# zxhuang1698/ZeroShape

Measured on AMD Instinct MI355X. Metric: sdf_query_points_per_sec_vox128, higher is better.
Workload: dtype f16x3

## Files before the change

### zeroshape_amd/csrc/sdf_decoder_split.hip

```cpp
#include "zs_common.h"
#include <stdlib.h>
#include "sdf_layout.h"
#include "sdf_math.h"
#include "zs_split16.h"
#include "sdf_query.h"
#include "../../include/zeroshape_hip.h"

#include <math.h>
#include <stdint.h>
#include <type_traits>

namespace {

using namespace zs::lay;
using namespace zs::qry;
using zs::dm::gelu_erf;
using zs::dm::softplus100;

typedef float f32x16 __attribute__((ext_vector_type(16)));
typedef float f32x4 __attribute__((ext_vector_type(4)));
typedef float f32x2 __attribute__((ext_vector_type(2)));
typedef unsigned u32x4 __attribute__((ext_vector_type(4)));

constexpr float S_GUARD = 64.0f;
constexpr int KB_U4 = 128;
constexpr int CK = 8;
constexpr int KPW = CK / WAVES;
constexpr int CHUNK_BYTES = CK * KB_U4 * 16;
constexpr int NBUF = 2;
constexpr int KB_TOTAL = G_TOTAL / 2;
constexpr int PRM_WINDOW = 4096;
constexpr int STAGE_FLOATS = NBUF * CHUNK_BYTES / 4;
constexpr int SLAB_TILES = NT - 1;
constexpr int SLAB_U4 = SLAB_TILES * 4 * 64;
constexpr int ZTILES_F4 = NT * 4 * 64;
static_assert(ZSLAB_F4 == 3 * ZTILES_F4, "the workspace slab holds three skip layers' feat partial products");
static_assert(B0_TABLE_FLOATS == PRM_WINDOW, "block0_window_kernel / block0_stream_kernel index an image's table by PRM_WINDOW");
constexpr int LDS_FLOATS = PRM_WINDOW + STAGE_FLOATS + WAVES * SLAB_U4 * 4;
static_assert(LDS_FLOATS * 4 == 160 * 1024, "the kernel owns the whole LDS of a CU");
static_assert(KB_TOTAL % CK == 0 && CK % WAVES == 0 && KPW * 2048 <= 4096, "chunking");
static_assert((RING * GROUP_FLOATS + PARAM_FLOATS) * 4 >= NBUF * CHUNK_BYTES, "prefetch stays inside the program");

constexpr int W_PP = P_PP;
constexpr int W_BLK = P_BLK0;
constexpr int W_IA = P_LNFG;
constexpr int W_IB = P_IMPL_PAIR + P_IMPL_PAIR_STRIDE;
static_assert(P_BLK_STRIDE <= PRM_WINDOW && W_IB - W_IA <= PRM_WINDOW && P_USED - W_IB <= PRM_WINDOW,
              "params windows");

#define DEV __device__ __forceinline__

DEV void pin(u32x4 &a, u32x4 &b) { asm volatile("" : "+v"(a), "+v"(b) : : "memory"); }

using zs::s16::mfma3;
using zs::s16::split2;

struct PT {
    u32x4 v[4];
};
template <typename T>
DEV PT pack_tile(const T &x) {
    PT p;
#pragma unroll
    for (int j = 0; j < 2; j++)
#pragma unroll
        for (int i = 0; i < 4; i++) {
            unsigned h, l;
            split2(x[8 * j + 2 * i], x[8 * j + 2 * i + 1], h, l);
            p.v[2 * j][i] = h;
            p.v[2 * j + 1][i] = l;
        }
    return p;
}

DEV void glds_kblocks(const char *gsrc, unsigned lds_dst) {
#ifdef ZS_EXP_NO_DMA
    if (gsrc != nullptr) return;
#endif
    asm volatile("s_mov_b32 m0, %1\n\ts_nop 0\n\tglobal_load_lds_dwordx4 %0, off"
                 "\n\tglobal_load_lds_dwordx4 %0, off offset:1024"
                 "\n\tglobal_load_lds_dwordx4 %0, off offset:2048"
                 "\n\tglobal_load_lds_dwordx4 %0, off offset:3072"
                 :
                 : "v"(gsrc), "s"(lds_dst)
                 : "memory");
}

struct AStream {
    const u32x4 *buf[NBUF];
    unsigned dst[NBUF];
    u32x4 hi, lo;
    const char *gsrc;

    DEV void init(const char *prog, u32x4 *stage, unsigned stage_addr, int wave, int lane) {
        const char *g = prog + wave * (KPW * KB_U4 * 16) + lane * 16;
        asm volatile("s_waitcnt vmcnt(0) lgkmcnt(0)\n\ts_barrier" ::: "memory");
#pragma unroll
        for (int i = 0; i < NBUF; i++) {
            buf[i] = stage + i * (CK * KB_U4) + lane;
            dst[i] = stage_addr + i * CHUNK_BYTES + wave * (KPW * KB_U4 * 16);
            glds_kblocks(g + i * CHUNK_BYTES, dst[i]);
        }
        gsrc = g + NBUF * CHUNK_BYTES;
        asm volatile("s_waitcnt vmcnt(4)\n\ts_barrier" ::: "memory");
        hi = buf[0][0];
        lo = buf[0][64];
    }
    template <int EXTRA_VM = 0>
    DEV void step(int pos, u32x4 &ahi, u32x4 &alo) {
        ahi = hi;
        alo = lo;
        if (pos == CK - 1) {
            static_assert(EXTRA_VM == 0 || EXTRA_VM == 4, "wait-count variants");
            if (EXTRA_VM == 4)
                asm volatile("s_waitcnt vmcnt(4) lgkmcnt(0)\n\ts_barrier" ::: "memory");
            else
                asm volatile("s_waitcnt vmcnt(0) lgkmcnt(0)\n\ts_barrier" ::: "memory");
            glds_kblocks(gsrc, dst[0]);
            gsrc += CHUNK_BYTES;
            const u32x4 *t = buf[0];
            const unsigned u = dst[0];
            buf[0] = buf[1];
            dst[0] = dst[1];
            buf[1] = t;
            dst[1] = u;
            hi = buf[0][0];
            lo = buf[0][64];
        } else {
#ifndef ZS_EXP_NO_AREAD
            hi = buf[0][(pos + 1) * KB_U4];
            lo = buf[0][(pos + 1) * KB_U4 + 64];
#endif
        }
    }
    DEV void seek(const char *base, int wave, int lane) { gsrc = base + wave * (KPW * KB_U4 * 16) + lane * 16; }
    DEV void drain() { asm volatile("s_waitcnt vmcnt(0) lgkmcnt(0)" ::: "memory"); }
};

struct Slab {
    u32x4 *fl;
    PT t7;
    DEV void store(int tile, const PT &p) {
        if (tile == SLAB_TILES) {
            t7 = p;
        } else {
#pragma unroll
            for (int q = 0; q < 4; q++) fl[(tile * 4 + q) * 64] = p.v[q];
        }
    }
};

DEV f32x16 zero16() {
    f32x16 v;
#pragma unroll
    for (int r = 0; r < 16; r++) v[r] = 0.f;
    return v;
}

struct NoSide {
    DEV void operator()(int, int) const {}
};
template <typename SIDE>
DEV void mfma3_gaps(f32x16 &acc, const u32x4 &ahi, const u32x4 &alo, const u32x4 &bhi, const u32x4 &blo, int kb,
                    SIDE &side) {
    using zs::s16::as_h;
    if (std::is_same<SIDE, NoSide>::value) {
        mfma3(acc, ahi, alo, bhi, blo);
        return;
    }
    acc = __builtin_amdgcn_mfma_f32_32x32x16_f16(as_h(alo), as_h(bhi), acc, 0, 0, 0);
    side(kb, 0);
    acc = __builtin_amdgcn_mfma_f32_32x32x16_f16(as_h(ahi), as_h(blo), acc, 0, 0, 0);
    side(kb, 1);
    acc = __builtin_amdgcn_mfma_f32_32x32x16_f16(as_h(ahi), as_h(bhi), acc, 0, 0, 0);
    side(kb, 2);
}

struct TilePacker {
    PT p;
    float prev;
    DEV void feed(int kb, float v) {
        if (kb & 1) {
            unsigned h, l;
            split2(prev, v, h, l);
            p.v[2 * (kb >> 3)][(kb & 7) >> 1] = h;
            p.v[2 * (kb >> 3) + 1][(kb & 7) >> 1] = l;
        }
        prev = v;
    }
};

struct GeluStager {
    float x, u, q, t, e, p;
    DEV void s0(float v) {
        x = v;
        u = fabsf(v) * 0.70710678118654752440f;
        q = (u * u) * -1.44269504088896340736f;
    }
    DEV void s1() { t = __builtin_amdgcn_rcpf(fmaf(0.3275911f, u, 1.0f)); }
    DEV void s2() {
        e = __builtin_amdgcn_exp2f(q);
        p = fmaf(0.75052702f, t, -1.02753365f);
    }
    DEV void s3() {
        p = fmaf(p, t, 1.00509130f);
        p = fmaf(p, t, -0.20116957f);
        p = fmaf(p, t, 0.18019173f);
        p = p * t;
        u = u * p;
    }
    DEV float s4() const { return fmaf(-u, e, fmaxf(x, 0.0f)); }
    DEV float all(float v) {
        s0(v); s1(); s2(); s3();
        return s4();
    }
    DEV void stage(int st, float v, int idx, TilePacker &pk) {
        if (st == 0) s0(v);
        else if (st == 1) s1();
        else if (st == 2) s2();
        else if (st == 3) s3();
        else if (st == 4) pk.feed(idx, s4());
    }
};
struct SoftplusStager {
    float x, t;
    DEV void s0(float v) {
        x = v;
        t = __builtin_amdgcn_exp2f(fabsf(v) * -144.26950408889634074f);
    }
    DEV void s1() { t = __builtin_amdgcn_logf(1.0f + t); }
    DEV float s2() const { return fmaf(t, 0.0069314718055994530942f, fmaxf(x, 0.0f)); }
};

#ifndef ZS_EXP_TWO_TERM
#define ZS_KBLOCK_MFMA_LO_HI "v_mfma_f32_32x32x16_f16 %[acc], %[alo], %[bh], %[acc]\n\t"
#else
#define ZS_KBLOCK_MFMA_LO_HI
#endif
#define ZS_KBLOCK_GELU(NAME, BREG, LEAD) \
DEV float NAME(f32x16 &acc, const u32x4 &ahi, const u32x4 &alo, const u32x4 &bhi, const u32x4 &blo, float x) {             \
    float u, q, d, t, e, m, p;                                                                                             \
    const float c0 = 0.70710678118654752440f, c1 = 0.3275911f, c2 = -1.02753365f;                                          \
    asm volatile(                                                                                                          \
                 LEAD ZS_KBLOCK_MFMA_LO_HI                                                                                 \
                 "v_mul_f32_e64 %[u], |%[x]|, %[c0]\n\t"                                                                   \
                 "v_mul_f32_e32 %[q], %[u], %[u]\n\t"                                                                      \
                 "v_mul_f32_e32 %[q], 0xbfb8aa3b, %[q]\n\t"                                                                \
                 "v_fma_f32 %[d], %[u], %[c1], 1.0\n\t"                                                                    \
                 "v_mfma_f32_32x32x16_f16 %[acc], %[ahi], %[bl], %[acc]\n\t"                                               \
                 "v_rcp_f32_e32 %[t], %[d]\n\t"                                                                            \
                 "v_exp_f32_e32 %[e], %[q]\n\t"                                                                            \
                 "v_max_f32_e32 %[m], 0, %[x]\n\t"                                                                         \
                 "v_mfma_f32_32x32x16_f16 %[acc], %[ahi], %[bh], %[acc]\n\t"                                               \
                 "v_fmamk_f32 %[p], %[t], 0x3f40228a, %[c2]\n\t"                                                           \
                 "v_fmaak_f32 %[p], %[p], %[t], 0x3f80a6d5\n\t"                                                            \
                 "v_fmaak_f32 %[p], %[p], %[t], 0xbe4dff65\n\t"                                                            \
                 "v_fmaak_f32 %[p], %[p], %[t], 0x3e38842e\n\t"                                                            \
                 "v_mul_f32_e64 %[p], %[t], -%[p]\n\t"                                                                     \
                 "v_mul_f32_e32 %[p], %[u], %[p]\n\t"                                                                      \
                 "v_fmac_f32_e32 %[m], %[p], %[e]"                                                                         \
                 : [acc] "+v"(acc), [u] "=&v"(u), [q] "=&v"(q), [d] "=&v"(d), [t] "=&v"(t), [e] "=&v"(e), [m] "=&v"(m),    \
                   [p] "=&v"(p)                                                                                            \
                 : [alo] "v"(alo), [ahi] "v"(ahi), [bh] BREG(bhi), [bl] BREG(blo), [x] "v"(x), [c0] "s"(c0), [c1] "s"(c1), \
                   [c2] "v"(c2));                                                                                          \
    return m;                                                                                                              \
}
ZS_KBLOCK_GELU(kblock_gelu, "v", "")
ZS_KBLOCK_GELU(kblock_gelu_breg, "a", "s_nop 1\n\t")
#undef ZS_KBLOCK_GELU
#undef ZS_KBLOCK_MFMA_LO_HI
DEV float kblock_softplus(f32x16 &acc, const u32x4 &ahi, const u32x4 &alo, const u32x4 &bhi, const u32x4 &blo, float x) {
    float t, m;
    const float c0 = -144.26950408889634074f;
    asm volatile(
#ifndef ZS_EXP_TWO_TERM
                 "v_mfma_f32_32x32x16_f16 %[acc], %[alo], %[bh], %[acc]\n\t"
#endif
                 "v_mul_f32_e64 %[t], |%[x]|, %[c0]\n\t"
                 "v_exp_f32_e32 %[t], %[t]\n\t"
                 "v_mfma_f32_32x32x16_f16 %[acc], %[ahi], %[bl], %[acc]\n\t"
                 "v_max_f32_e32 %[m], 0, %[x]\n\t"
                 "v_add_f32_e32 %[t], 1.0, %[t]\n\t"
                 "v_log_f32_e32 %[t], %[t]\n\t"
                 "v_mfma_f32_32x32x16_f16 %[acc], %[ahi], %[bh], %[acc]\n\t"
                 "s_nop 0\n\t"
                 "v_fmac_f32_e32 %[m], 0x3be32166, %[t]"
                 : [acc] "+v"(acc), [t] "=&v"(t), [m] "=&v"(m)
                 : [alo] "v"(alo), [ahi] "v"(ahi), [bh] "v"(bhi), [bl] "v"(blo), [x] "v"(x), [c0] "s"(c0));
    return m;
}

DEV void mfma_settle(f32x16 &acc) { asm volatile("s_nop 7\n\ts_nop 3" : "+v"(acc)); }

template <int KT, int EXTRA_VM = 0, typename SIDE = NoSide>
DEV void gemm_reg(AStream &s, const PT *X, f32x16 &acc, SIDE side = SIDE()) {
#pragma unroll
    for (int kt = 0; kt < KT; kt++)
#pragma unroll
        for (int j = 0; j < 2; j++) {
            u32x4 ahi, alo;
            s.step((kt * 2 + j) & (CK - 1), ahi, alo);
            pin(ahi, alo);
            mfma3_gaps(acc, ahi, alo, X[kt].v[2 * j], X[kt].v[2 * j + 1], kt * 2 + j, side);
        }
}
template <typename SIDE>
DEV void mfma3_breg(f32x16 &acc, const u32x4 &ahi, const u32x4 &alo, const u32x4 &bhi, const u32x4 &blo, int kb,
                    SIDE &side) {
    asm volatile("s_nop 1\n\tv_mfma_f32_32x32x16_f16 %0, %1, %2, %0" : "+v"(acc) : "v"(alo), "a"(bhi));
    side(kb, 0);
    asm volatile("s_nop 1\n\tv_mfma_f32_32x32x16_f16 %0, %1, %2, %0" : "+v"(acc) : "v"(ahi), "a"(blo));
    side(kb, 1);
    asm volatile("s_nop 1\n\tv_mfma_f32_32x32x16_f16 %0, %1, %2, %0" : "+v"(acc) : "v"(ahi), "a"(bhi));
    side(kb, 2);
}
template <int KT, typename SIDE = NoSide>
DEV void gemm_areg(AStream &s, const PT *X, f32x16 &acc, SIDE side = SIDE()) {
#pragma unroll
    for (int kt = 0; kt < KT; kt++)
#pragma unroll
        for (int j = 0; j < 2; j++) {
            u32x4 ahi, alo;
            s.step((kt * 2 + j) & (CK - 1), ahi, alo);
            pin(ahi, alo);
            mfma3_breg(acc, ahi, alo, X[kt].v[2 * j], X[kt].v[2 * j + 1], kt * 2 + j, side);
        }
}
template <typename SIDE>
DEV void mfma3_cacc(f32x16 &acc, const u32x4 &ahi, const u32x4 &alo, const u32x4 &bhi, const u32x4 &blo, int kb,
                    SIDE &side) {
    asm volatile("s_nop 1\n\tv_mfma_f32_32x32x16_f16 %0, %1, %2, %0" : "+a"(acc) : "v"(alo), "v"(bhi));
    side(kb, 0);
    asm volatile("s_nop 1\n\tv_mfma_f32_32x32x16_f16 %0, %1, %2, %0" : "+a"(acc) : "v"(ahi), "v"(blo));
    side(kb, 1);
    asm volatile("s_nop 1\n\tv_mfma_f32_32x32x16_f16 %0, %1, %2, %0" : "+a"(acc) : "v"(ahi), "v"(bhi));
    side(kb, 2);
}
template <bool YACC = false, typename SIDE = NoSide, int NKB = 2>
DEV void gemm_one(AStream &s, const PT &X, f32x16 &acc, int pos0, int kb0 = 0, SIDE side = SIDE()) {
#pragma unroll
    for (int j = 0; j < NKB; j++) {
        u32x4 ahi, alo;
        s.step((pos0 + j) & (CK - 1), ahi, alo);
        pin(ahi, alo);
        if (YACC)
            mfma3_cacc(acc, ahi, alo, X.v[2 * j], X.v[2 * j + 1], kb0 + j, side);
        else
            mfma3_gaps(acc, ahi, alo, X.v[2 * j], X.v[2 * j + 1], kb0 + j, side);
    }
}
DEV void slab_b(const Slab &sl, int kb, u32x4 &bh, u32x4 &bl) {
    if (kb >= SLAB_TILES * 2) {
        bh = sl.t7.v[(kb & 1) * 2];
        bl = sl.t7.v[(kb & 1) * 2 + 1];
    } else {
        bh = sl.fl[kb * KB_U4];
        bl = sl.fl[kb * KB_U4 + 64];
    }
}
template <typename SIDE = NoSide>
DEV void gemm_lds(AStream &s, const Slab &sl, f32x16 &acc, int pos0 = 0, SIDE side = SIDE()) {
    u32x4 bh, bl;
    slab_b(sl, 0, bh, bl);
#pragma unroll
    for (int kb = 0; kb < NT * 2; kb++) {
        u32x4 ahi, alo;
        s.step((pos0 + kb) & (CK - 1), ahi, alo);
        u32x4 nh = bh, nl = bl;
        if (kb + 1 < NT * 2) slab_b(sl, kb + 1, nh, nl);
        pin(ahi, alo);
        mfma3_gaps(acc, ahi, alo, bh, bl, kb, side);
        bh = nh;
        bl = nl;
    }
}

template <int ACT, typename FIN, typename TAIL>
DEV void gemm_lds_act(AStream &s, const Slab &sl, f32x16 &acc, const f32x16 &cur, FIN fin, TAIL tail) {
    u32x4 bh, bl;
    slab_b(sl, 0, bh, bl);
#pragma unroll
    for (int kb = 0; kb < NT * 2; kb++) {
        u32x4 ahi, alo;
        s.step(kb & (CK - 1), ahi, alo);
        u32x4 nh = bh, nl = bl;
        if (kb + 1 < NT * 2) slab_b(sl, kb + 1, nh, nl);
        const float r = ACT == 0 ? kblock_gelu(acc, ahi, alo, bh, bl, cur[kb]) : kblock_softplus(acc, ahi, alo, bh, bl, cur[kb]);
        bh = nh;
        bl = nl;
        fin(kb, r);
        tail(kb);
    }
}
template <int ACT, typename FIN, typename TAIL>
DEV void gemm_reg_act(AStream &s, const PT *X, f32x16 &acc, const f32x16 &cur, FIN fin, TAIL tail) {
#pragma unroll
    for (int kt = 0; kt < NT; kt++)
#pragma unroll
        for (int j = 0; j < 2; j++) {
            u32x4 ahi, alo;
            const int kb = kt * 2 + j;
            s.step(kb & (CK - 1), ahi, alo);
            const float r = ACT == 0 ? kblock_gelu(acc, ahi, alo, X[kt].v[2 * j], X[kt].v[2 * j + 1], cur[kb])
                                     : kblock_softplus(acc, ahi, alo, X[kt].v[2 * j], X[kt].v[2 * j + 1], cur[kb]);
            fin(kb, r);
            tail(kb);
        }
}
template <typename FIN, typename TAIL>
DEV void gemm_areg_gelu(AStream &s, const PT *X, f32x16 &acc, const f32x16 &cur, FIN fin, TAIL tail) {
#pragma unroll
    for (int kt = 0; kt < NT; kt++)
#pragma unroll
        for (int j = 0; j < 2; j++) {
            u32x4 ahi, alo;
            const int kb = kt * 2 + j;
            s.step(kb & (CK - 1), ahi, alo);
            const float r = kblock_gelu_breg(acc, ahi, alo, X[kt].v[2 * j], X[kt].v[2 * j + 1], cur[kb]);
            fin(kb, r);
            tail(kb);
        }
}

#ifndef ZS_SPLIT_PERMLANE
DEV float half_sum(float v) { return v + __shfl_xor(v, 32, 64); }
DEV float half_max(float v) { return fmaxf(v, __shfl_xor(v, 32, 64)); }
#else
DEV void half_pair(float v, float &lo, float &hi) {
    lo = v;
    hi = v;
    asm volatile("s_nop 4\n\tv_permlane32_swap_b32 %0, %1\n\ts_nop 4" : "+v"(lo), "+v"(hi));
}
DEV float half_sum(float v) {
    float lo, hi;
    half_pair(v, lo, hi);
    return lo + hi;
}
#ifdef ZS_SPLIT_PERMLANE_SUM_ONLY
DEV float half_max(float v) { return fmaxf(v, __shfl_xor(v, 32, 64)); }
#else
DEV float half_max(float v) {
    float lo, hi;
    half_pair(v, lo, hi);
    return fmaxf(lo, hi);
}
#endif
#endif

DEV void rp(const float *prm, int off, int tile, int hi, float *v) {
    const f32x4 *q = reinterpret_cast<const f32x4 *>(prm + off + tile * 32 + hi * 16);
#pragma unroll
    for (int i = 0; i < 4; i++) {
        const f32x4 a = q[i];
        v[4 * i + 0] = a.x; v[4 * i + 1] = a.y; v[4 * i + 2] = a.z; v[4 * i + 3] = a.w;
    }
}
DEV f32x16 rp16(const float *prm, int off, int tile, int hi) {
    float t[16];
    rp(prm, off, tile, hi, t);
    f32x16 v;
#pragma unroll
    for (int r = 0; r < 16; r++) v[r] = t[r];
    return v;
}
constexpr int B0_BPROJ = 0, B0_C = 256, B0_T = 1024;
static_assert(B0_T + HEADS * 3 * 128 == PRM_WINDOW, "the block-0 table is exactly one params window");
constexpr float B0S_LO_SCALE = 64.0f;
constexpr int B0S_KB_HEAD = 34;
static_assert(B0_STREAM_KB == HEADS * B0S_KB_HEAD && B0_STREAM_KB % CK == 0 && B0_STREAM_BYTES == (size_t)B0_STREAM_KB * KB_U4 * 16,
              "the compact stream is whole chunks");
static_assert(B0S_KB_HEAD == 5 + (2 * LT - 1) + 2 * NT && L - 32 * (LT - 1) <= 16, "latent tile 6: rows 16-31 are padding");
DEV void rem2(unsigned h, float a, float b, float &ra, float &rb) {
    asm("v_fma_mix_f32 %0, %1, -1.0, %2 op_sel_hi:[1,0,0]" : "=v"(ra) : "v"(h), "v"(a));
    asm("v_fma_mix_f32 %0, %1, -1.0, %2 op_sel:[1,0,0] op_sel_hi:[1,0,0]" : "=v"(rb) : "v"(h), "v"(b));
}
DEV u32x4 rank5_b(float u0, float u1, float u2, float u3, int hi, bool &bad) {
    using zs::s16::pk_f16;
    const unsigned lim = 0x477fe000u;
    bad = (__builtin_bit_cast(unsigned, u0) & 0x7fffffffu) > lim || (__builtin_bit_cast(unsigned, u1) & 0x7fffffffu) > lim ||
          (__builtin_bit_cast(unsigned, u2) & 0x7fffffffu) > lim || (__builtin_bit_cast(unsigned, u3) & 0x7fffffffu) > lim;
    const unsigned h01 = pk_f16(u0, u1), h23 = pk_f16(u2, u3);
    float r0, r1, r2, r3;
    rem2(h01, u0, u1, r0, r1);
    rem2(h23, u2, u3, r2, r3);
    const float s = B0S_LO_SCALE, is = 1.0f / B0S_LO_SCALE;
    const unsigned l01 = pk_f16(r0 * s, r1 * s), l23 = pk_f16(r2 * s, r3 * s);
    const unsigned d01 = pk_f16((u0 - r0) * is, (u1 - r1) * is), d23 = pk_f16((u2 - r2) * is, (u3 - r3) * is);
    static_assert(B0S_LO_SCALE == 64.0f, "ud4's bit pattern");
    return hi ? u32x4{d01, d23, 0x00003c00u, 0x00002400u} : u32x4{h01, h23, l01, l23};
}
DEV f32x16 mfma_rank5(const u32x4 &a, const u32x4 &ub) {
    return __builtin_amdgcn_mfma_f32_32x32x16_f16(zs::s16::as_h(a), zs::s16::as_h(ub), zero16(), 0, 0, 0);
}

DEV f32x16 xyz_affine(const float *prm, int off, int tile, int hi, float x, float y, float z) {
    const f32x4 *q = reinterpret_cast<const f32x4 *>(prm + off + tile * 128 + hi * 64);
    f32x16 v;
#pragma unroll
    for (int r = 0; r < 16; r++) {
        const f32x4 w = q[r];
        v[r] = fmaf(w.z, z, fmaf(w.y, y, fmaf(w.x, x, w.w)));
    }
    return v;
}

struct XyzInit {
    const f32x4 *q;
    f32x4 w;
    f32x16 v;
    DEV void start(const float *prm, int off, int tile, int hi) {
        q = reinterpret_cast<const f32x4 *>(prm + off + tile * 128 + hi * 64);
        w = q[0];
    }
    DEV void step(int r, float x, float y, float z) {
        v[r] = fmaf(w.z, z, fmaf(w.y, y, fmaf(w.x, x, w.w)));
        if (r + 1 < 16) w = q[r + 1];
    }
};
struct RowInit {
    const f32x4 *q;
    f32x4 w;
    f32x16 v;
    DEV void start(const float *prm, int off, int tile, int hi) {
        q = reinterpret_cast<const f32x4 *>(prm + off + tile * 32 + hi * 16);
        w = q[0];
    }
    DEV void step(int r) {
        if ((r & 3) == 0) {
            v[r] = w.x; v[r + 1] = w.y; v[r + 2] = w.z; v[r + 3] = w.w;
            if (r + 4 < 16) w = q[(r >> 2) + 1];
        }
    }
};

DEV void ln_stats(const f32x16 *x, float &mean, float &rstd) {
    float s = 0.f;
#pragma unroll
    for (int kt = 0; kt < NT; kt++)
#pragma unroll
        for (int r = 0; r < 16; r++) s += x[kt][r];
    s = half_sum(s);
    mean = s * (1.0f / 256.0f);
    float v = 0.f;
#pragma unroll
    for (int kt = 0; kt < NT; kt++)
#pragma unroll
        for (int r = 0; r < 16; r++) {
            const float d = x[kt][r] - mean;
            v = fmaf(d, d, v);
        }
    v = half_sum(v);
    rstd = 1.0f / sqrtf(v * (1.0f / 256.0f) + 1e-6f);
}
DEV void layer_norm_lds(const f32x16 *x, Slab &sl, const float *prm, int g_off, int b_off, int hi) {
    float mean, rstd;
    ln_stats(x, mean, rstd);
#pragma unroll
    for (int kt = 0; kt < NT; kt++) {
        float g[16], b[16], t[16];
        rp(prm, g_off, kt, hi, g);
        rp(prm, b_off, kt, hi, b);
#pragma unroll
        for (int r = 0; r < 16; r++) t[r] = fmaf((x[kt][r] - mean) * rstd, g[r], b[r]);
        sl.store(kt, pack_tile(t));
    }
}
#ifndef ZS_SPLIT_LN_SLAB
constexpr bool LN2_REGS = true;
#else
constexpr bool LN2_REGS = false;
#endif
DEV void layer_norm_reg(const f32x16 *x, PT *xn, const float *prm, int g_off, int b_off, int hi) {
    float mean, rstd;
    ln_stats(x, mean, rstd);
#pragma unroll
    for (int kt = 0; kt < NT; kt++) {
        float g[16], b[16], t[16];
        rp(prm, g_off, kt, hi, g);
        rp(prm, b_off, kt, hi, b);
#pragma unroll
        for (int r = 0; r < 16; r++) t[r] = fmaf((x[kt][r] - mean) * rstd, g[r], b[r]);
        xn[kt] = pack_tile(t);
#pragma unroll
        for (int q = 0; q < 4; q++) asm volatile("" : "+a"(xn[kt].v[q]));
    }
}

DEV void load_params(float *prm, const float *prog_params, int start, int count) {
    __syncthreads();
    const f32x4 *src = reinterpret_cast<const f32x4 *>(prog_params + start);
    f32x4 *dst = reinterpret_cast<f32x4 *>(prm);
    for (int i = threadIdx.x; i < count / 4; i += WAVES * 64) dst[i] = src[i];
    __syncthreads();
}

template <bool MASK, int NKB = 2>
DEV void softmax_pv(AStream &s, f32x16 &S, f32x16 &o, float &m_run, float &z_run, float c, int hi, int pos0) {
    float mt = -INFINITY;
#pragma unroll
    for (int r = 0; r < 16; r++) {
        if (MASK) {
            const int rw = (r & 3) + 8 * (r >> 2) + 4 * hi;
            S[r] = rw < L - 32 * (LT - 1) ? S[r] : -INFINITY;
        }
        mt = fmaxf(mt, S[r]);
    }
    mt *= c;
    constexpr float LAZY = 8.0f;
    if (__builtin_amdgcn_ballot_w64(mt > m_run + LAZY) != 0) {
        mt = half_max(mt);
        const float m_new = fmaxf(m_run, mt);
        const float alpha = __builtin_amdgcn_exp2f(m_run - m_new);
        z_run *= alpha;
#pragma unroll
        for (int r = 0; r < 16; r++) o[r] *= alpha;
        m_run = m_new;
    }
    float zs_ = 0.f;
#pragma unroll
    for (int r = 0; r < 16; r++) {
        const float p = __builtin_amdgcn_exp2f(fmaf(S[r], c, -m_run));
        S[r] = p;
        zs_ += p;
    }
    z_run += zs_;
    gemm_one<false, NoSide, NKB>(s, pack_tile(S), o, pos0);
}
template <bool MASK>
DEV void attn_tile(AStream &s, const PT &q, f32x16 &o, float &m_run, float &z_run, float c, int hi,
                   int pos0) {
    f32x16 S = zero16();
    gemm_one(s, q, S, pos0);
    softmax_pv<MASK>(s, S, o, m_run, z_run, c, hi, pos0 + 2);
}

DEV void merge_self(f32x16 &o, const f32x16 &v, float m_run, float z_run, float s_self) {
    const float m_new = fmaxf(m_run, s_self);
    const float alpha = __builtin_amdgcn_exp2f(m_run - m_new);
    const float p_self = __builtin_amdgcn_exp2f(s_self - m_new);
    const float z = fmaf(half_sum(z_run), alpha, p_self);
    const float inv = 1.0f / z;
    const float a_i = alpha * inv, p_i = p_self * inv;
#pragma unroll
    for (int r = 0; r < 16; r++) o[r] = fmaf(p_i, v[r], o[r] * a_i);
}

#ifdef ZS_EXP_TIMING
#define ZS_STAMP(i) do { if (dbg) dbg[i] = __builtin_amdgcn_s_memtime(); } while (0)
#else
#define ZS_STAMP(i) do { } while (0)
#endif
DEV float decode_tile(const char *prog, float *prm, u32x4 *stage, unsigned stage_addr, u32x4 *slab,
                      const char *b0s, float px, float py, float pz, int wave, int lane, float &guard,
                      unsigned long long *dbg) {
    const int hi = lane >> 5;
    const float *prog_params = reinterpret_cast<const float *>(prog) + REC_FLOATS;
    AStream s;
    s.init(b0s ? b0s : prog, stage, stage_addr, wave, lane);
    Slab sl;
    sl.fl = slab;
    ZS_STAMP(0);

    load_params(prm, prog_params, W_PP, 1024);
    f32x16 y[NT];
#pragma unroll
    for (int kt = 0; kt < NT; kt++) y[kt] = xyz_affine(prm, 0, kt, hi, px, py, pz);

    ZS_STAMP(1);

    const float scale = 0.17677669529663688110f;

#pragma unroll 1
    for (int blk = 0; blk < BLOCKS; blk++) {
        const bool strm = blk == 0 && b0s != nullptr;
        float rstd0 = 0.f;
        u32x4 ub = {0u, 0u, 0u, 0u};
        bool u_bad = false;
        if (strm) {
            load_params(prm, prog_params, W_BLK, P_BLK_STRIDE);
            float mean;
            ln_stats(y, mean, rstd0);
            ub = rank5_b(px * rstd0, py * rstd0, pz * rstd0, rstd0, hi, u_bad);
        } else {
            load_params(prm, prog_params, W_BLK + blk * P_BLK_STRIDE, P_BLK_STRIDE);
            layer_norm_lds(y, sl, prm, PB_LN1G, PB_LN1B, hi);
        }
        ZS_STAMP(2 + blk * 4);
#pragma unroll
        for (int nt = 0; nt < NT; nt++) y[nt] += rp16(prm, PB_BPROJ, nt, hi);

        auto head = [&](int hd, auto Ptag) {
            constexpr int P = decltype(Ptag)::value;
            f32x16 q = rp16(prm, PB_BQKV, hd * 3 + 0, hi);
            gemm_lds(s, sl, q, P);
            f32x16 k = rp16(prm, PB_BQKV, hd * 3 + 1, hi);
            gemm_lds(s, sl, k, P);
            f32x16 v = rp16(prm, PB_BQKV, hd * 3 + 2, hi);
            gemm_lds(s, sl, v, P);

            const float c = scale * 1.44269504088896340736f;
            float s_self = 0.f;
            float qq = 0.f;
#pragma unroll
            for (int r = 0; r < 16; r++) {
                s_self = fmaf(q[r], k[r], s_self);
                qq = fmaf(q[r], q[r], qq);
            }
            s_self = half_sum(s_self) * c;
            {
                const float km = prog_params[P_KMAX + blk * HEADS + hd] * scale;
                guard = fmaxf(guard, half_sum(qq) * (km * km));
            }
            const PT qp = pack_tile(q);

            float m_run = -INFINITY, z_run = 0.f;
            f32x16 o = zero16();
#pragma unroll
            for (int l2 = 0; l2 < (LT - 1) / 2; l2++) {
                attn_tile<false>(s, qp, o, m_run, z_run, c, hi, P);
                attn_tile<false>(s, qp, o, m_run, z_run, c, hi, (P + 4) & (CK - 1));
            }
            attn_tile<true>(s, qp, o, m_run, z_run, c, hi, P);
            merge_self(o, v, m_run, z_run, s_self);
            const PT op = pack_tile(o);
#pragma unroll
            for (int nt = 0; nt < NT; nt++) gemm_one(s, op, y[nt], (P + 4 + 2 * nt) & (CK - 1));
        };
        auto head_b0s = [&](int hd, auto Ptag) {
            constexpr int P = decltype(Ptag)::value;
            u32x4 a0, a1;
            s.step(P & (CK - 1), a0, a1);
            pin(a0, a1);
            const f32x16 q = mfma_rank5(a0, ub), k = mfma_rank5(a1, ub);
            s.step((P + 1) & (CK - 1), a0, a1);
            pin(a0, a1);
            const f32x16 v = mfma_rank5(a0, ub);
            f32x16 S = mfma_rank5(a1, ub);
            float s_self = 0.f, qq = 0.f;
#pragma unroll
            for (int r = 0; r < 16; r++) {
                s_self = fmaf(q[r], k[r], s_self);
                qq = fmaf(q[r], q[r], qq);
            }
            s_self = half_sum(s_self) * (scale * 1.44269504088896340736f);
            {
                const float km = prog_params[P_KMAX + hd] * scale;
                guard = fmaxf(guard, half_sum(qq) * (km * km));
            }
            float m_run = -INFINITY, z_run = 0.f;
            f32x16 o = zero16();
            softmax_pv<false>(s, S, o, m_run, z_run, 1.0f, hi, P + 2);
#pragma unroll
            for (int i = 0; i < (LT - 1) / 2; i++) {
                s.step((P + 4 + 5 * i) & (CK - 1), a0, a1);
                pin(a0, a1);
                S = mfma_rank5(a0, ub);
                softmax_pv<false>(s, S, o, m_run, z_run, 1.0f, hi, P + 5 + 5 * i);
                S = mfma_rank5(a1, ub);
                if (2 * i + 2 < LT - 1)
                    softmax_pv<false>(s, S, o, m_run, z_run, 1.0f, hi, P + 7 + 5 * i);
                else
                    softmax_pv<true, 1>(s, S, o, m_run, z_run, 1.0f, hi, P + 7 + 5 * i);
            }
            merge_self(o, v, m_run, z_run, s_self);
            const PT op = pack_tile(o);
            if (P == 6 && hd == HEADS - 1) s.seek(prog + HEADS * (G_HEAD / 2) * (KB_U4 * 16), wave, lane);
#pragma unroll
            for (int nt = 0; nt < NT; nt++) gemm_one(s, op, y[nt], (P + 18 + 2 * nt) & (CK - 1));
        };
        static_assert((LT - 1) % 2 == 0 && (3 * NT * 2 + LT * 4 + NT * 2) % CK == 4, "head = 11.5 chunks");
        static_assert(B0S_KB_HEAD % CK == 2 && HEADS % 4 == 0 && (HEADS * (G_HEAD / 2)) % CK == 0,
                      "compact heads start at chunk positions 0, 2, 4, 6; the program resumes on a chunk boundary");
        if (strm) {
#pragma unroll 1
            for (int hd = 0; hd < HEADS; hd += 4) {
                head_b0s(hd, std::integral_constant<int, 0>());
                head_b0s(hd + 1, std::integral_constant<int, 2>());
                head_b0s(hd + 2, std::integral_constant<int, 4>());
                head_b0s(hd + 3, std::integral_constant<int, 6>());
            }
            guard = __builtin_bit_cast(float, u_bad ? 0x7f800000u : __builtin_bit_cast(unsigned, guard));
        } else {
#pragma unroll 1
            for (int hd = 0; hd < HEADS; hd += 2) {
                head(hd, std::integral_constant<int, 0>());
                head(hd + 1, std::integral_constant<int, 4>());
            }
        }

        ZS_STAMP(3 + blk * 4);
        PT xn[NT];
        if constexpr (LN2_REGS)
            layer_norm_reg(y, xn, prm, PB_LN2G, PB_LN2B, hi);
        else
            layer_norm_lds(y, sl, prm, PB_LN2G, PB_LN2B, hi);
#pragma unroll
        for (int nt = 0; nt < NT; nt++) y[nt] += rp16(prm, PB_B2, nt, hi);
        ZS_STAMP(4 + blk * 4);
        RowInit bi;
        f32x16 hid = rp16(prm, PB_B1, 0, hi);
        bi.start(prm, PB_B1, 1, hi);
        auto bias_side = [&](int kb, int g) {
            if (g == 2 && (kb & 3) == 1) bi.step(kb & ~3);
        };
        if constexpr (LN2_REGS) {
            gemm_areg<NT>(s, xn, hid, bias_side);
            mfma_settle(hid);
        } else {
            gemm_lds(s, sl, hid, 0, bias_side);
        }
#pragma unroll 1
        for (int ht = 0; ht < HT - 1; ht++) {
            f32x16 nxt = bi.v;
            bi.start(prm, PB_B1, ht + 2 < HT ? ht + 2 : HT - 1, hi);
            TilePacker e;
            auto fin = [&](int kb, float r) { e.feed(kb, r); };
            auto tail = [&](int kb) { if ((kb & 3) == 1) bi.step(kb & ~3); };
            if constexpr (LN2_REGS)
                gemm_areg_gelu(s, xn, nxt, hid, fin, tail);
            else
                gemm_lds_act<0>(s, sl, nxt, hid, fin, tail);
#pragma unroll
            for (int nt = 0; nt < NT; nt++) gemm_one(s, e.p, y[nt], (2 * nt) & (CK - 1));
            hid = nxt;
        }
        {
#pragma unroll
            for (int r = 0; r < 16; r++) hid[r] = gelu_erf(hid[r]);
            const PT hp = pack_tile(hid);
#pragma unroll
            for (int nt = 0; nt < NT; nt++) gemm_one(s, hp, y[nt], (2 * nt) & (CK - 1));
        }
        ZS_STAMP(5 + blk * 4);
    }

    load_params(prm, prog_params, W_IA, W_IB - W_IA);
    float h[NT * 16];
    {
        float mean, rstd;
        ln_stats(y, mean, rstd);
#pragma unroll
        for (int kt = 0; kt < NT; kt++) {
            float g[16], b[16];
            rp(prm, P_LNFG - W_IA, kt, hi, g);
            rp(prm, P_LNFB - W_IA, kt, hi, b);
#pragma unroll
            for (int r = 0; r < 16; r++) h[kt * 16 + r] = fmaf((y[kt][r] - mean) * rstd, g[r], b[r]);
        }
    }
    ZS_STAMP(10);
    PT hp[NT];

#pragma unroll
    for (int kt = 0; kt < NT; kt++) hp[kt] = pack_tile(h + kt * 16);
    {
        f32x16 prev;
        XyzInit ini;
        ini.v = xyz_affine(prm, P_IMPL0 - W_IA, 0, hi, px, py, pz);
#pragma unroll
        for (int nt = 0; nt <= NT; nt++) {
            TilePacker e;
            if (nt < NT) {
                f32x16 acc = ini.v;
                if (nt + 1 < NT) ini.start(prm, P_IMPL0 - W_IA, nt + 1, hi);
                if (nt > 0)
                    gemm_reg_act<1>(s, hp, acc, prev, [&](int kb, float r) { e.feed(kb, r); },
                                    [&](int kb) { if (nt + 1 < NT) ini.step(kb, px, py, pz); });
                else
                    gemm_reg<NT, 0>(s, hp, acc, [&](int kb, int g) { if (g == 2) ini.step(kb, px, py, pz); });
                if (nt > 0) sl.store(nt - 1, e.p);
                prev = acc;
            } else {
                mfma_settle(prev);
#pragma unroll
                for (int kb = 0; kb < 16; kb++) e.feed(kb, softplus100(prev[kb]));
                sl.store(nt - 1, e.p);
            }
        }
    }
    ZS_STAMP(11);
    const float rsqrt2 = 0.70710678118654752440f;
    PT fp[NT];
#pragma unroll
    for (int kt = 0; kt < NT; kt++) {
        float t[16];
#pragma unroll
        for (int r = 0; r < 16; r++) t[r] = h[kt * 16 + r] * rsqrt2;
        fp[kt] = pack_tile(t);
    }
    const float sx = px * rsqrt2, sy = py * rsqrt2, sz = pz * rsqrt2;

    ZS_STAMP(12);
    {
        f32x16 prev;
        RowInit ini;
        ini.v = rp16(prm, P_IMPL1 - W_IA, 0, hi);
#pragma unroll
        for (int nt = 0; nt <= NT; nt++) {
            TilePacker e;
            if (nt < NT) {
                f32x16 acc = ini.v;
                if (nt + 1 < NT) ini.start(prm, P_IMPL1 - W_IA, nt + 1, hi);
                if (nt > 0)
                    gemm_lds_act<1>(s, sl, acc, prev, [&](int kb, float r) { e.feed(kb, r * rsqrt2); },
                                    [&](int kb) { if (nt + 1 < NT) ini.step(kb); });
                else
                    gemm_lds(s, sl, acc, 0, [&](int kb, int g) { if (g == 2) ini.step(kb); });
                if (nt > 0) hp[nt - 1] = e.p;
                prev = acc;
            } else {
                mfma_settle(prev);
#pragma unroll
                for (int kb = 0; kb < 16; kb++) e.feed(kb, softplus100(prev[kb]) * rsqrt2);
                hp[nt - 1] = e.p;
            }
        }
    }
    ZS_STAMP(13);
    float out = 0.f;
#pragma unroll 1
    for (int i = 0; i < 3; i++) {
        if (i == 1) load_params(prm, prog_params, W_IB, P_USED - W_IB);
        const int pp = i == 0 ? P_IMPL_PAIR - W_IA : (i - 1) * P_IMPL_PAIR_STRIDE;
        {
            f32x16 prev;
            XyzInit ini;
            ini.v = xyz_affine(prm, pp, 0, hi, sx, sy, sz);
#pragma unroll
            for (int nt = 0; nt <= NT; nt++) {
                TilePacker e;
                if (nt > 0) mfma_settle(prev);
                if (nt < NT) {
                    f32x16 acc = ini.v;
                    if (nt + 1 < NT) ini.start(prm, pp, nt + 1, hi);
                    if (nt > 0)
                        gemm_reg_act<1>(s, hp, acc, prev, [&](int kb, float r) { e.feed(kb, r); }, [&](int) {});
                    else
                        gemm_reg<NT>(s, hp, acc);
                    gemm_areg<NT>(s, fp, acc, [&](int kb, int g) {
                        if (g == 2 && nt + 1 < NT) ini.step(kb, sx, sy, sz);
                    });
                    if (nt > 0) sl.store(nt - 1, e.p);
                    prev = acc;
                } else {
#pragma unroll
                    for (int kb = 0; kb < 16; kb++) e.feed(kb, softplus100(prev[kb]));
                    sl.store(nt - 1, e.p);
                }
            }
        }
        const float post = i < 2 ? rsqrt2 : 1.0f;
        {
            f32x16 prev;
            RowInit ini, w8;
            const float wsel = i == 2 ? 1.0f : 0.0f;
            ini.v = rp16(prm, pp + 1024, 0, hi);
#pragma unroll
            for (int r = 0; r < 16; r++) w8.v[r] = 0.f;
#pragma unroll
            for (int nt = 0; nt <= NT; nt++) {
                TilePacker e;
                const f32x16 w = w8.v * wsel;
                auto finish = [&](int kb, float v) {
                    const float t = v * post;
                    e.feed(kb, t);
                    out = fmaf(t, w[kb], out);
                };
                if (nt < NT) {
                    f32x16 acc = ini.v;
                    if (nt + 1 < NT) ini.start(prm, pp + 1024, nt + 1, hi);
                    w8.start(prm, P_W8 - W_IB, nt, hi);
                    auto tail = [&](int kb) {
                        if (nt + 1 < NT) ini.step(kb);
                        w8.step(kb);
                    };
                    if (nt > 0)
                        gemm_lds_act<1>(s, sl, acc, prev, [&](int kb, float r) { finish(kb, r); }, tail);
                    else
                        gemm_lds(s, sl, acc, 0, [&](int kb, int g) { if (g == 2) tail(kb); });
                    if (nt > 0) hp[nt - 1] = e.p;
                    prev = acc;
                } else {
                    mfma_settle(prev);
#pragma unroll
                    for (int kb = 0; kb < 16; kb++) finish(kb, softplus100(prev[kb]));
                    hp[nt - 1] = e.p;
                }
            }
        }
    }
    ZS_STAMP(14);
    s.drain();
    out = half_sum(out);
    ZS_STAMP(15);
    return out + prm[P_B8 - W_IB];
}

template <bool GRID>
__global__ __launch_bounds__(WAVES * 64, 1) void sdf_decode_split_kernel(
    const char *__restrict__ programs, size_t program_stride_bytes, int batch,
    const float *__restrict__ points,
    const float *__restrict__ axis,
    int G, long long first_point,
    int m,
    float *__restrict__ out, int apply_sigmoid, f32x4 *__restrict__ workspace,
    int *__restrict__ tile_flags,
    int static_order,
    const char *__restrict__ block0_streams) {
    __shared__ __attribute__((aligned(16))) float lds[LDS_FLOATS];
    float *prm = lds;
    const int lane = threadIdx.x & 63;
    const int wave = __builtin_amdgcn_readfirstlane(threadIdx.x >> 6);
    u32x4 *stage = reinterpret_cast<u32x4 *>(lds + PRM_WINDOW);
    const unsigned stage_addr = __builtin_amdgcn_readfirstlane(
        (unsigned)(uintptr_t)(__attribute__((address_space(3))) float *)(lds + PRM_WINDOW));
    u32x4 *fl = reinterpret_cast<u32x4 *>(lds + PRM_WINDOW + STAGE_FLOATS) + wave * SLAB_U4 + lane;

    const int tiles_per_img = (m + PTS_PER_BLOCK - 1) / PTS_PER_BLOCK;
    const int total = tiles_per_img * batch;
    int *tile_counter = zs::qry::tile_counter(workspace);
    int *tile_slot = tile_counter + 16 + blockIdx.x;
    const int dyn_tiles = total > (int)gridDim.x ? total - (int)gridDim.x : 0;
    for (int tile = blockIdx.x;;) {
      if (tile < total) {
        const int img = tile / tiles_per_img;
        const int t = tile - img * tiles_per_img;
        const char *prog = programs + (size_t)img * program_stride_bytes;

        const int p = t * PTS_PER_BLOCK + wave * PTS_PER_WAVE + (lane & 31);
        const int pc = p < m ? p : m - 1;
        float px, py, pz;
        if (GRID) {
            const long long gp = first_point + pc;
            const long long gg = (long long)G * G;
            const int ix = (int)(gp / gg);
            const int rem = (int)(gp - (long long)ix * gg);
            const int iy = rem / G;
            const int iz = rem - iy * G;
            px = axis[ix];
            py = axis[iy];
            pz = axis[iz];
        } else {
            const float *q = points + ((size_t)img * m + pc) * 3;
            px = q[0];
            py = q[1];
            pz = q[2];
        }
#ifdef ZS_EXP_TIMING
        unsigned long long *dbg = (blockIdx.x == 0 && threadIdx.x == 0 && tile == 0)
            ? timing_stamps(workspace) : nullptr;
#else
        unsigned long long *dbg = nullptr;
#endif
        float guard = 0.f;
        const char *b0s = block0_streams ? block0_streams + (size_t)img * B0_STREAM_BYTES : nullptr;
        float logit = decode_tile(prog, prm, stage, stage_addr, fl, b0s, px, py, pz, wave, lane, guard, dbg);
        if (apply_sigmoid) logit = 1.0f / (1.0f + expf(-logit));
        const unsigned bad = reinterpret_cast<const unsigned *>(prog)[REC_FLOATS + P_FLAG];
        const bool pt_bad = (__builtin_bit_cast(unsigned, px) & 0x7f800000u) == 0x7f800000u ||
                            (__builtin_bit_cast(unsigned, py) & 0x7f800000u) == 0x7f800000u ||
                            (__builtin_bit_cast(unsigned, pz) & 0x7f800000u) == 0x7f800000u;
        if (bad || pt_bad) logit = __builtin_bit_cast(float, 0x7fc00000u);
        if (tile_flags) {
            const bool over = !(__builtin_bit_cast(unsigned, guard) <= __builtin_bit_cast(unsigned, S_GUARD * S_GUARD));
            if (__builtin_amdgcn_ballot_w64(over || bad != 0) != 0 && lane == 0) tile_flags[tile] = 1;
        }
        if (lane < 32 && p < m) out[(size_t)img * m + p] = logit;
      }
        if (static_order) {
            tile += (int)gridDim.x;
            if (tile >= total) break;
            continue;
        }
        if (threadIdx.x == 0) {
            const int d = __hip_atomic_fetch_add(tile_counter, 1, __ATOMIC_RELAXED, __HIP_MEMORY_SCOPE_AGENT);
            if (d == dyn_tiles + (int)gridDim.x - 1)
                __hip_atomic_store(tile_counter, 0, __ATOMIC_RELAXED, __HIP_MEMORY_SCOPE_AGENT);
            __hip_atomic_store(tile_slot, d, __ATOMIC_RELAXED, __HIP_MEMORY_SCOPE_AGENT);
        }
        __syncthreads();
        const int d = __builtin_amdgcn_readfirstlane(__hip_atomic_load(tile_slot, __ATOMIC_RELAXED, __HIP_MEMORY_SCOPE_AGENT));
        if ((unsigned)d >= (unsigned)dyn_tiles) break;
        tile = (int)gridDim.x + d;
    }
}

DEV bool out_of_range(const f32x4 &v) {
    const unsigned lim = 0x477fe000u;
    return (__builtin_bit_cast(unsigned, v.x) & 0x7fffffffu) > lim || (__builtin_bit_cast(unsigned, v.y) & 0x7fffffffu) > lim ||
           (__builtin_bit_cast(unsigned, v.z) & 0x7fffffffu) > lim || (__builtin_bit_cast(unsigned, v.w) & 0x7fffffffu) > lim;
}

__host__ __device__ inline int split_source_kblock(int kb) {
    constexpr int KB_BLOCK = G_BLOCK / 2, KB_ATT = HEADS * G_HEAD / 2;
    static_assert(KB_BLOCK - KB_ATT == HT * 32, "an MLP section is 32 K-blocks per hidden tile");
    constexpr int KB_IMPL0 = BLOCKS * KB_BLOCK, KB_L = NT * NT * 2;
    if (kb >= KB_IMPL0 + G_IMPL / 2) return kb;
    if (kb >= KB_IMPL0) {
        const int p = kb - KB_IMPL0;
        if (p < KB_L) return kb;
        if (p < 2 * KB_L) return KB_IMPL0 + 4 * KB_L + (p - KB_L);
        const int q = p - 2 * KB_L, pair = q / (3 * KB_L), r = q - pair * 3 * KB_L;
        if (r >= 2 * KB_L) return KB_IMPL0 + (5 + 2 * pair + 1) * KB_L + (r - 2 * KB_L);
        const int nt = r / (4 * NT), w = r - nt * 4 * NT;
        return w < 2 * NT ? KB_IMPL0 + (5 + 2 * pair) * KB_L + nt * 2 * NT + w
                          : KB_IMPL0 + (1 + pair) * KB_L + nt * 2 * NT + (w - 2 * NT);
    }
    const int blk = kb / KB_BLOCK, p = kb - blk * KB_BLOCK - KB_ATT;
    if (p < 16) return kb;
    const int q = p - 16, it = q >> 5, r = q & 31;
    int src;
    if (it < HT - 1)
        src = r < 16 ? (it + 1) * 32 + r : it * 32 + r;
    else
        src = it * 32 + 16 + r;
    return blk * KB_BLOCK + KB_ATT + src;
}

__global__ __launch_bounds__(256) void split_program_kernel(const float *__restrict__ src,
                                                            size_t src_stride_floats,
                                                            u32x4 *__restrict__ dst,
                                                            size_t dst_stride_u4) {
    const int img = blockIdx.y;
    const float *s = src + (size_t)img * src_stride_floats;
    u32x4 *d = dst + (size_t)img * dst_stride_u4;
    const int e = blockIdx.x * 256 + threadIdx.x;
    constexpr int REC_KB = REC_FLOATS / (KB_U4 * 4);
    if (e < REC_KB * 64) {
        const int kb = e >> 6, lane = e & 63;
        const f32x4 *g = reinterpret_cast<const f32x4 *>(s) + (size_t)split_source_kblock(kb) * 128;
        const f32x4 a = g[lane], b = g[64 + lane];
        if (out_of_range(a) || out_of_range(b)) atomicOr(reinterpret_cast<unsigned *>(d) + REC_FLOATS + P_FLAG, 1u);
// ... 305 lines not shown
```

Before: 83.79 million.

## Keep implicit-layer odd activations in VGPR/AGPR registers instead of LDS slab

Implicit-network intermediate activations (odd layers) are now kept in register tiles, part in VGPRs and the rest in AGPRs, instead of being written to and read back from the LDS slab. The feature tile fp is packed earlier and pinned to AGPRs. New softplus and gelu MFMA variants take B operands from AGPRs. This removes LDS store/load traffic and its waits, but raises register pressure and may cause spills or lower occupancy.

```diff
diff --git a/zeroshape_amd/csrc/sdf_decoder_split.hip b/zeroshape_amd/csrc/sdf_decoder_split.hip
--- a/zeroshape_amd/csrc/sdf_decoder_split.hip
+++ b/zeroshape_amd/csrc/sdf_decoder_split.hip
@@ -31,8 +31,19 @@
 constexpr int KB_TOTAL = G_TOTAL / 2;
 constexpr int PRM_WINDOW = 4096;
 constexpr int STAGE_FLOATS = NBUF * CHUNK_BYTES / 4;
+#ifndef ZS_SPLIT_IMPL_SLAB
+constexpr bool IMPL_REGS = true;
+#else
+constexpr bool IMPL_REGS = false;
+#endif
+#ifndef ZS_SPLIT_LN_SLAB
+constexpr bool LN2_REGS = true;
+#else
+constexpr bool LN2_REGS = false;
+#endif
 constexpr int SLAB_TILES = NT - 1;
 constexpr int SLAB_U4 = SLAB_TILES * 4 * 64;
+constexpr int SLAB_USED = IMPL_REGS && LN2_REGS ? SLAB_TILES - 1 : SLAB_TILES;
 constexpr int ZTILES_F4 = NT * 4 * 64;
 static_assert(ZSLAB_F4 == 3 * ZTILES_F4, "the workspace slab holds three skip layers' feat partial products");
 static_assert(B0_TABLE_FLOATS == PRM_WINDOW, "block0_window_kernel / block0_stream_kernel index an image's table by PRM_WINDOW");
@@ -139,10 +150,10 @@
 
 struct Slab {
     u32x4 *fl;
-    PT t7;
+    PT tr[NT - SLAB_USED];
     DEV void store(int tile, const PT &p) {
-        if (tile == SLAB_TILES) {
-            t7 = p;
+        if (tile >= SLAB_USED) {
+            tr[tile - SLAB_USED] = p;
         } else {
 #pragma unroll
             for (int q = 0; q < 4; q++) fl[(tile * 4 + q) * 64] = p.v[q];
@@ -268,27 +279,29 @@
 ZS_KBLOCK_GELU(kblock_gelu, "v", "")
 ZS_KBLOCK_GELU(kblock_gelu_breg, "a", "s_nop 1\n\t")
 #undef ZS_KBLOCK_GELU
+#define ZS_KBLOCK_SOFTPLUS(NAME, BREG, LEAD) \
+DEV float NAME(f32x16 &acc, const u32x4 &ahi, const u32x4 &alo, const u32x4 &bhi, const u32x4 &blo, float x) {             \
+    float t, m;                                                                                                            \
+    const float c0 = -144.26950408889634074f;                                                                              \
+    asm volatile(                                                                                                          \
+                 LEAD ZS_KBLOCK_MFMA_LO_HI                                                                                 \
+                 "v_mul_f32_e64 %[t], |%[x]|, %[c0]\n\t"                                                                   \
+                 "v_exp_f32_e32 %[t], %[t]\n\t"                                                                            \
+                 "v_mfma_f32_32x32x16_f16 %[acc], %[ahi], %[bl], %[acc]\n\t"                                               \
+                 "v_max_f32_e32 %[m], 0, %[x]\n\t"                                                                         \
+                 "v_add_f32_e32 %[t], 1.0, %[t]\n\t"                                                                       \
+                 "v_log_f32_e32 %[t], %[t]\n\t"                                                                            \
+                 "v_mfma_f32_32x32x16_f16 %[acc], %[ahi], %[bh], %[acc]\n\t"                                               \
+                 "s_nop 0\n\t"                                                                                             \
+                 "v_fmac_f32_e32 %[m], 0x3be32166, %[t]"                                                                   \
+                 : [acc] "+v"(acc), [t] "=&v"(t), [m] "=&v"(m)                                                             \
+                 : [alo] "v"(alo), [ahi] "v"(ahi), [bh] BREG(bhi), [bl] BREG(blo), [x] "v"(x), [c0] "s"(c0));              \
+    return m;                                                                                                              \
+}
+ZS_KBLOCK_SOFTPLUS(kblock_softplus, "v", "")
+ZS_KBLOCK_SOFTPLUS(kblock_softplus_breg, "a", "s_nop 1\n\t")
+#undef ZS_KBLOCK_SOFTPLUS
 #undef ZS_KBLOCK_MFMA_LO_HI
-DEV float kblock_softplus(f32x16 &acc, const u32x4 &ahi, const u32x4 &alo, const u32x4 &bhi, const u32x4 &blo, float x) {
-    float t, m;
-    const float c0 = -144.26950408889634074f;
-    asm volatile(
-#ifndef ZS_EXP_TWO_TERM
-                 "v_mfma_f32_32x32x16_f16 %[acc], %[alo], %[bh], %[acc]\n\t"
-#endif
-                 "v_mul_f32_e64 %[t], |%[x]|, %[c0]\n\t"
-                 "v_exp_f32_e32 %[t], %[t]\n\t"
-                 "v_mfma_f32_32x32x16_f16 %[acc], %[ahi], %[bl], %[acc]\n\t"
-                 "v_max_f32_e32 %[m], 0, %[x]\n\t"
-                 "v_add_f32_e32 %[t], 1.0, %[t]\n\t"
-                 "v_log_f32_e32 %[t], %[t]\n\t"
-                 "v_mfma_f32_32x32x16_f16 %[acc], %[ahi], %[bh], %[acc]\n\t"
-                 "s_nop 0\n\t"
-                 "v_fmac_f32_e32 %[m], 0x3be32166, %[t]"
-                 : [acc] "+v"(acc), [t] "=&v"(t), [m] "=&v"(m)
-                 : [alo] "v"(alo), [ahi] "v"(ahi), [bh] "v"(bhi), [bl] "v"(blo), [x] "v"(x), [c0] "s"(c0));
-    return m;
-}
 
 DEV void mfma_settle(f32x16 &acc) { asm volatile("s_nop 7\n\ts_nop 3" : "+v"(acc)); }
 
@@ -314,7 +327,7 @@
     asm volatile("s_nop 1\n\tv_mfma_f32_32x32x16_f16 %0, %1, %2, %0" : "+v"(acc) : "v"(ahi), "a"(bhi));
     side(kb, 2);
 }
-template <int KT, typename SIDE = NoSide>
+template <int KT, int VT = 0, typename SIDE = NoSide>
 DEV void gemm_areg(AStream &s, const PT *X, f32x16 &acc, SIDE side = SIDE()) {
 #pragma unroll
     for (int kt = 0; kt < KT; kt++)
@@ -323,7 +336,10 @@
             u32x4 ahi, alo;
             s.step((kt * 2 + j) & (CK - 1), ahi, alo);
             pin(ahi, alo);
-            mfma3_breg(acc, ahi, alo, X[kt].v[2 * j], X[kt].v[2 * j + 1], kt * 2 + j, side);
+            if (kt < VT)
+                mfma3_gaps(acc, ahi, alo, X[kt].v[2 * j], X[kt].v[2 * j + 1], kt * 2 + j, side);
+            else
+                mfma3_breg(acc, ahi, alo, X[kt].v[2 * j], X[kt].v[2 * j + 1], kt * 2 + j, side);
         }
 }
 template <typename SIDE>
@@ -350,9 +366,9 @@
     }
 }
 DEV void slab_b(const Slab &sl, int kb, u32x4 &bh, u32x4 &bl) {
-    if (kb >= SLAB_TILES * 2) {
-        bh = sl.t7.v[(kb & 1) * 2];
-        bl = sl.t7.v[(kb & 1) * 2 + 1];
+    if (kb >= SLAB_USED * 2) {
+        bh = sl.tr[(kb >> 1) - SLAB_USED].v[(kb & 1) * 2];
+        bl = sl.tr[(kb >> 1) - SLAB_USED].v[(kb & 1) * 2 + 1];
     } else {
         bh = sl.fl[kb * KB_U4];
         bl = sl.fl[kb * KB_U4 + 64];
@@ -407,8 +423,8 @@
             tail(kb);
         }
 }
-template <typename FIN, typename TAIL>
-DEV void gemm_areg_gelu(AStream &s, const PT *X, f32x16 &acc, const f32x16 &cur, FIN fin, TAIL tail) {
+template <int ACT, int VT = 0, typename FIN, typename TAIL>
+DEV void gemm_areg_act(AStream &s, const PT *X, f32x16 &acc, const f32x16 &cur, FIN fin, TAIL tail) {
 #pragma unroll
     for (int kt = 0; kt < NT; kt++)
 #pragma unroll
@@ -416,7 +432,10 @@
             u32x4 ahi, alo;
             const int kb = kt * 2 + j;
             s.step(kb & (CK - 1), ahi, alo);
-            const float r = kblock_gelu_breg(acc, ahi, alo, X[kt].v[2 * j], X[kt].v[2 * j + 1], cur[kb]);
+            const u32x4 &bh = X[kt].v[2 * j], &bl = X[kt].v[2 * j + 1];
+            const float r = kt < VT ? (ACT == 0 ? kblock_gelu(acc, ahi, alo, bh, bl, cur[kb]) : kblock_softplus(acc, ahi, alo, bh, bl, cur[kb]))
+                                    : (ACT == 0 ? kblock_gelu_breg(acc, ahi, alo, bh, bl, cur[kb])
+                                                : kblock_softplus_breg(acc, ahi, alo, bh, bl, cur[kb]));
             fin(kb, r);
             tail(kb);
         }
@@ -565,11 +584,6 @@
         sl.store(kt, pack_tile(t));
     }
 }
-#ifndef ZS_SPLIT_LN_SLAB
-constexpr bool LN2_REGS = true;
-#else
-constexpr bool LN2_REGS = false;
-#endif
 DEV void layer_norm_reg(const f32x16 *x, PT *xn, const float *prm, int g_off, int b_off, int hi) {
     float mean, rstd;
     ln_stats(x, mean, rstd);
@@ -817,7 +831,7 @@
             auto fin = [&](int kb, float r) { e.feed(kb, r); };
             auto tail = [&](int kb) { if ((kb & 3) == 1) bi.step(kb & ~3); };
             if constexpr (LN2_REGS)
-                gemm_areg_gelu(s, xn, nxt, hid, fin, tail);
+                gemm_areg_act<0>(s, xn, nxt, hid, fin, tail);
             else
                 gemm_lds_act<0>(s, sl, nxt, hid, fin, tail);
 #pragma unroll
@@ -849,7 +863,36 @@
         }
     }
     ZS_STAMP(10);
+    constexpr int IMPL_VT = 2;
     PT hp[NT];
+    PT hq[NT];
+    const float rsqrt2 = 0.70710678118654752440f;
+    PT fp[NT];
+    auto make_fp = [&]() {
+#pragma unroll
+        for (int kt = 0; kt < NT; kt++) {
+            float t[16];
+#pragma unroll
+            for (int r = 0; r < 16; r++) t[r] = h[kt * 16 + r] * rsqrt2;
+            fp[kt] = pack_tile(t);
+            if constexpr (IMPL_REGS) {
+#pragma unroll
+                for (int q = 0; q < 4; q++) asm volatile("" : "+a"(fp[kt].v[q]));
+            }
+        }
+    };
+    if constexpr (IMPL_REGS) make_fp();
+    auto to_odd = [&](int tile, const PT &p) {
+        if constexpr (IMPL_REGS) {
+            hq[tile] = p;
+            if (tile >= IMPL_VT) {
+#pragma unroll
+                for (int q = 0; q < 4; q++) asm volatile("" : "+a"(hq[tile].v[q]));
+            }
+        } else {
+            sl.store(tile, p);
+        }
+    };
 
 #pragma unroll
     for (int kt = 0; kt < NT; kt++) hp[kt] = pack_tile(h + kt * 16);
@@ -868,26 +911,18 @@
                                     [&](int kb) { if (nt + 1 < NT) ini.step(kb, px, py, pz); });
                 else
                     gemm_reg<NT, 0>(s, hp, acc, [&](int kb, int g) { if (g == 2) ini.step(kb, px, py, pz); });
-                if (nt > 0) sl.store(nt - 1, e.p);
+                if (nt > 0) to_odd(nt - 1, e.p);
                 prev = acc;
             } else {
                 mfma_settle(prev);
 #pragma unroll
                 for (int kb = 0; kb < 16; kb++) e.feed(kb, softplus100(prev[kb]));
-                sl.store(nt - 1, e.p);
+                to_odd(nt - 1, e.p);
             }
         }
     }
     ZS_STAMP(11);
-    const float rsqrt2 = 0.70710678118654752440f;
-    PT fp[NT];
-#pragma unroll
-    for (int kt = 0; kt < NT; kt++) {
-        float t[16];
-#pragma unroll
-        for (int r = 0; r < 16; r++) t[r] = h[kt * 16 + r] * rsqrt2;
-        fp[kt] = pack_tile(t);
-    }
+    if constexpr (!IMPL_REGS) make_fp();
     const float sx = px * rsqrt2, sy = py * rsqrt2, sz = pz * rsqrt2;
 
     ZS_STAMP(12);
@@ -901,11 +936,22 @@
             if (nt < NT) {
                 f32x16 acc = ini.v;
                 if (nt + 1 < NT) ini.start(prm, P_IMPL1 - W_IA, nt + 1, hi);
-                if (nt > 0)
-                    gemm_lds_act<1>(s, sl, acc, prev, [&](int kb, float r) { e.feed(kb, r * rsqrt2); },
-                                    [&](int kb) { if (nt + 1 < NT) ini.step(kb); });
-                else
-                    gemm_lds(s, sl, acc, 0, [&](int kb, int g) { if (g == 2) ini.step(kb); });
+                auto fin = [&](int kb, float r) { e.feed(kb, r * rsqrt2); };
+                auto tail = [&](int kb) { if (nt + 1 < NT) ini.step(kb); };
+                auto side = [&](int kb, int g) { if (g == 2) ini.step(kb); };
+                if constexpr (IMPL_REGS) {
+                    if (nt > 0) {
+                        mfma_settle(prev);
+                        gemm_areg_act<1, IMPL_VT>(s, hq, acc, prev, fin, tail);
+                    } else {
+                        gemm_areg<NT, IMPL_VT>(s, hq, acc, side);
+                    }
+                } else {
+                    if (nt > 0)
+                        gemm_lds_act<1>(s, sl, acc, prev, fin, tail);
+                    else
+                        gemm_lds(s, sl, acc, 0, side);
+                }
                 if (nt > 0) hp[nt - 1] = e.p;
                 prev = acc;
             } else {
@@ -940,12 +986,12 @@
                     gemm_areg<NT>(s, fp, acc, [&](int kb, int g) {
                         if (g == 2 && nt + 1 < NT) ini.step(kb, sx, sy, sz);
                     });
-                    if (nt > 0) sl.store(nt - 1, e.p);
+                    if (nt > 0) to_odd(nt - 1, e.p);
                     prev = acc;
                 } else {
 #pragma unroll
                     for (int kb = 0; kb < 16; kb++) e.feed(kb, softplus100(prev[kb]));
-                    sl.store(nt - 1, e.p);
+                    to_odd(nt - 1, e.p);
                 }
             }
         }
@@ -974,10 +1020,20 @@
                         if (nt + 1 < NT) ini.step(kb);
                         w8.step(kb);
                     };
-                    if (nt > 0)
-                        gemm_lds_act<1>(s, sl, acc, prev, [&](int kb, float r) { finish(kb, r); }, tail);
-                    else
-                        gemm_lds(s, sl, acc, 0, [&](int kb, int g) { if (g == 2) tail(kb); });
+                    auto side = [&](int kb, int g) { if (g == 2) tail(kb); };
+                    if constexpr (IMPL_REGS) {
+                        if (nt > 0) {
+                            mfma_settle(prev);
+                            gemm_areg_act<1, IMPL_VT>(s, hq, acc, prev, finish, tail);
+                        } else {
+                            gemm_areg<NT, IMPL_VT>(s, hq, acc, side);
+                        }
+                    } else {
+                        if (nt > 0)
+                            gemm_lds_act<1>(s, sl, acc, prev, finish, tail);
+                        else
+                            gemm_lds(s, sl, acc, 0, side);
+                    }
                     if (nt > 0) hp[nt - 1] = e.p;
                     prev = acc;
                 } else {
```

Result: faster. 84.83 million, median of 6 (+1.2%).
